# mym-br/gama_tts

Hardware: AMD Instinct MI355X
Metric: audio samples/sec (whole node), batched VTM @44.1kHz (higher is better)
Workload: dtype f32

## Files before the change

__graft_entry__.py:

```python
import os
import subprocess
import sys

ROOT = os.path.dirname(os.path.abspath(__file__))
for p in (ROOT, os.path.join(ROOT, "tests")):
    if p not in sys.path:
        sys.path.insert(0, p)


def build():
    env = dict(os.environ)
    subprocess.run(["make", "-C", os.path.join(ROOT, "gama_tts_amd", "csrc"), "ARCH=gfx950"], check=True, env=env)
    subprocess.run(["make", "-C", os.path.join(ROOT, "oracle"), "oracle"], check=True, env=env)
    subprocess.run(["make", "-C", os.path.join(ROOT, "oracle"), "ref"], check=True, env=env)
    import gama_tts_amd

    gama_tts_amd.load_library()


def smoke():
    import numpy as np

    import gama_tts_amd as g
    import oracle
    import tracks

    params = tracks.random_tracks(4, 25, seed0=42, consonant_heavy=True)
    cfgd = g.read_config_file(oracle.VOICE_MALE)
    plan = g.Plan(g.config_from_dict(cfgd, 44100.0, 1), 250.0, 0)
    audio, counts, maxabs = plan.synthesize_host(params)
    ref = oracle.synthesize_batch(oracle.male_config(44100.0, 1), params)
    assert audio.shape == ref.shape and (counts == ref.shape[1]).all(), (audio.shape, ref.shape, counts)
    err = float(np.abs(audio.astype(np.float64) - ref).max() / np.abs(ref).max())
    assert err < 2e-7, err
    assert np.allclose(maxabs, np.abs(audio).max(axis=1))
    from gama_tts_amd import capi
    plan32 = g.Plan(g.config_from_dict(cfgd, 44100.0, 1, capi.PRECISION_F32), 250.0, 0)
    audio32, _, _ = plan32.synthesize_host(params)
    ref32 = oracle.synthesize_batch(oracle.male_config(44100.0, 1, float_model=1), params)
    assert np.array_equal(audio32, ref32)
    plan5 = g.Plan(g.config5_from_dict(g.read_config_file(oracle.VOICE5_MALE)), 250.0, 0)
    audio5, counts5, _ = plan5.synthesize_host(params[:2])
    err5 = 0.0
    for b in range(2):
        ref5, _ = oracle.synthesize5(oracle.male5_config(48000.0), params[b])
        assert counts5[b] == ref5.size
        err5 = max(err5, float(np.abs(audio5[b, : ref5.size].astype(np.float64) - ref5).max() / np.abs(ref5).max()))
    assert err5 < 2e-6, err5
    plan5f = g.Plan(g.config5_from_dict(g.read_config_file(oracle.VOICE5_MALE), None, capi.PRECISION_F32), 250.0, 0, float_model5=True)
    audio5f, counts5f, _ = plan5f.synthesize_host(params[:2])
    for b in range(2):
        ref5f, _ = oracle.synthesize5(oracle.male5_config(48000.0, 1), params[b])
        assert counts5f[b] == ref5f.size and np.array_equal(audio5f[b, : ref5f.size], ref5f)
    print("smoke ok: batch=4 frames=25 samples=%d fp64 peak-relative error %.3g, float path bit-identical, model 5 error %.3g, "
          "float model 5 bit-identical" % (ref.shape[1], err, err5))


if __name__ == "__main__":
    build()
    if len(sys.argv) > 1 and sys.argv[1] == "smoke":
        smoke()
```

gama_tts_amd/capi.py:

```python
import ctypes
import os

import numpy as np

_HERE = os.path.dirname(os.path.abspath(__file__))
_LIB_NAME = "libgama_vtm.so"
N_PARAM = 16
DEVICE_NONE = -1
PRECISION_F64 = 0
PRECISION_MIXED = 1
PRECISION_F32 = 2
TUBE_10_6 = 0
TUBE_30_18 = 1
TABLE_FIR, TABLE_SRC_H, TABLE_SRC_DH, TABLE_WAVETABLE = 0, 1, 2, 3
_STATUS_UNSUPPORTED = 4


class GvtmError(RuntimeError):
    def __init__(self, status, message):
        super().__init__("gvtm status %d: %s" % (status, message))
        self.status = status


class Config(ctypes.Structure):
# ... 118 lines not shown
        "gvtm_plan_reserve": (i, [vp, sz]),
        "gvtm_host_alloc": (i, [sz, vp]),
        "gvtm_host_free": (None, [vp]),
        "gvtm_stream_create": (i, [vp, sz, vp]),
        "gvtm_stream_create_voices": (i, [vp, vp, sz, vp]),
        "gvtm_stream_destroy": (None, [vp]),
        "gvtm_stream_reset": (i, [vp]),
        "gvtm_stream_reset_voices": (i, [vp, vp]),
        "gvtm_stream_capacity": (sz, [vp, sz]),
        "gvtm_stream_push": (i, [vp, vp, vp, sz, vp, sz, vp]),
        "gvtm_stream_finish": (i, [vp, vp, sz, vp, vp]),
        "gvtm_normalize_batch_device": (i, [vp, vp, sz, sz, vp, vp, vp, vp, vp, vp]),
        "gvtm_plan_set_timing": (i, [vp, i]),
        "gvtm_plan_take_kernel_ms": (dbl, [vp, vp]),
        "gvtm_tracks_frame_count": (sz, [tracks, vp, sz]),
        "gvtm_generate_tracks_device": (i, [i, tracks, vp, vp, sz, sz, vp, vp, vp, vp]),
        "gvtm_synthesize_events_device": (i, [vp, tracks, vp, vp, sz, sz, vp, sz, vp, vp, vp, vp, vp]),
        "gvtm_plan_set_voice_tracks": (i, [vp, tracks, sz]),
        "gvtm_generate_tracks_voices_device": (i, [vp, vp, vp, vp, sz, sz, vp, vp, vp, vp]),
        "gvtm_synthesize_events_voices_device": (i, [vp, vp, vp, vp, sz, sz, vp, sz, vp, vp, vp, vp, vp]),
        "gvtm_tracks_chunks_frame_count": (sz, [tracks, vp, vp, sz]),
        "gvtm_generate_tracks_chunks_device": (i, [vp, vp, vp, vp, vp, sz, sz, vp, vp, vp, vp]),
        "gvtm_synthesize_events_chunks_device": (i, [vp, vp, vp, vp, vp, sz, sz, vp, sz, vp, vp, vp, vp, vp]),
        "gvtm_intonation_apply_host": (i64, [tracks, vp, sz, vp, sz, vp, sz, vp]),
        "gvtm_apply_intonation_device": (i, [vp, vp, vp, sz, vp, vp, vp, vp, sz, vp, sz, vp, vp, vp]),
        "gvtm_synthesize_intonation_device": (i, [vp, vp, vp, sz, vp, vp, vp, vp, sz, sz, sz, vp, sz, vp, vp, vp, vp, vp, vp]),
        "gvtm_modification_filter_length": (i64, [vp, i]),
        "gvtm_modification_apply_host": (i, [vp, i, vp, sz, vp, vp, sz, vp, vp, vp, vp]),
        "gvtm_apply_modifications_device": (i, [vp, vp, vp, sz, vp, vp, vp, vp, vp, vp, vp, sz, sz, vp, vp, vp, vp]),
        "gvtm_synthesize_modified_device": (i, [vp, vp, vp, sz, vp, vp, vp, vp, vp, vp, vp, sz, sz, vp, sz, vp, vp, vp, vp, vp]),
        "gvtm_targets_filter_length": (i64, [vp, i]),
        "gvtm_targets_output_count": (sz, [vp, sz]),
        "gvtm_targets_output_capacity": (sz, [vp, sz]),
        "gvtm_targets_apply_host": (i, [vp, i, vp, vp, vp, i64, vp, vp]),
        "gvtm_targets_apply_host_from": (i, [vp, i, vp, vp, vp, i64, i64, vp, vp, vp]),
        "gvtm_synthesize_targets_device": (i, [vp, vp, sz, vp, vp, vp, vp, sz, sz, vp, sz, vp, vp, vp, vp]),
        "gvtm_stream_push_targets": (i, [vp, vp, vp, vp, vp, sz, vp, sz, vp, vp]),
        "gvtm_stream_targets_capacity": (sz, [vp, sz]),
        "gvtm_stream_targets_points": (i, [vp, vp]),
        "gvtm_stream_push_events": (i, [vp, vp, vp, vp, vp, sz, vp, vp]),
        "gvtm_stream_get_drift": (i, [vp, vp]),
        "gvtm_stream_set_drift": (i, [vp, vp]),
        "gvtm_events_packed_layout": (sz, [vp, vp, vp, vp, vp, sz, vp, vp]),
        "gvtm_synthesize_events_packed_host": (i, [vp, vp, vp, vp, vp, sz, vp, sz, vp, vp, vp, sz, vp, vp, vp]),
        "gvtm_synthesize_events_packed_host_pcm16": (i, [vp, vp, vp, vp, vp, sz, vp, sz, vp, vp, vp, sz, vp, vp, vp, vp]),
        "gvtm_generate_tracks_host": (i, [i, tracks, vp, vp, sz, sz, vp, vp, vp]),
    }
    hooks = {
        "gvtm_debug_set_rows": (i, [vp, i]),
        "gvtm_debug_lds_bytes": (sz, [vp, i]),
        "gvtm_debug_launch_shape": (i, [vp, sz, i, vp]),
        "gvtm_debug_stream_launch_shape": (i, [vp, sz, vp]),
        "gvtm_debug_chunk_length": (i, [vp, sz]),
        "gvtm_debug_fir_literals": (i, [vp]),
        "gvtm_debug_plan_fir_literals": (i, [vp]),
        "gvtm_debug_force_generic_fir": (i, [vp]),
        "gvtm_debug_plan_src_phases": (i, [vp]),
        "gvtm_debug_plan_src_phase_table": (i, [vp, vp, sz]),
        "gvtm_debug_force_generic_src": (i, [vp]),
        "gvtm_debug_plan_static_wavetable": (i, [vp]),
        "gvtm_debug_force_dynamic_wavetable": (i, [vp]),
        "gvtm_debug_noise_table": (i, [sz, i, vp]),
        "gvtm_debug_set_taps": (i, [vp, vp]),
        "gvtm_debug_set_phase_cycles": (i, [vp, vp]),
        "gvtm_debug_dpp_selftest": (i, [vp, vp]),
        "gvtm_debug_short_math": (i, [i, vp, sz, vp]),
        "gvtm_debug_device_float_math": (i, [vp, i, vp, sz, vp]),
        "gvtm_debug_group_voices": (i, [vp, vp, sz, i, vp, vp, vp, vp]),
        "gvtm_debug_tracks_append": (i, [vp, vp, vp, vp, vp, vp, sz, sz, vp, vp, vp]),
        "gvtm_debug_tracks_slice": (i, [vp, vp, i64, vp, vp, vp, vp, sz, sz, vp, vp, vp, vp]),
        "gvtm_debug_carry_rows": (i, [vp, vp, vp, vp, sz, sz]),
    }
    return product, hooks


PROTOTYPES, HOOK_PROTOTYPES = _prototypes()
_REQUIRED = (
    "gvtm_status_string", "gvtm_last_error", "gvtm_device_count", "gvtm_plan_create", "gvtm_plan_create_model5", "gvtm_plan_destroy",
    "gvtm_plan_info", "gvtm_plan_table", "gvtm_output_count", "gvtm_output_capacity", "gvtm_synthesize_batch_device",
    "gvtm_synthesize_batch_host", "gvtm_synthesize_batch_host_pcm16", "gvtm_host_alloc", "gvtm_host_free", "gvtm_normalize_batch_device",
    "gvtm_tracks_frame_count", "gvtm_generate_tracks_device", "gvtm_synthesize_events_device", "gvtm_generate_tracks_host",
    "gvtm_stream_create", "gvtm_stream_destroy", "gvtm_stream_reset", "gvtm_stream_capacity", "gvtm_stream_push", "gvtm_stream_finish",
    "gvtm_plan_set_timing", "gvtm_plan_take_kernel_ms")


def library_path(diagnostics=False):
    return os.path.join(_HERE, "lib", "libgama_vtm_diag.so" if diagnostics else _LIB_NAME)


_libs = {}


def load_library(diagnostics=False):
    if diagnostics in _libs:
        return _libs[diagnostics]
    path = (os.environ.get("GVTM_DIAG_LIBRARY") or library_path(True)) if diagnostics else (os.environ.get("GVTM_LIBRARY") or library_path())
    try:
        import torch
    except ImportError:
        pass
    if not os.path.exists(path):
        raise ImportError("%s is missing: run `python -c 'import __graft_entry__ as g; g.build()'` "
                          "(make -C gama_tts_amd/csrc). There is no fallback path." % path)
    lib = ctypes.CDLL(path)
    table = {**PROTOTYPES, **HOOK_PROTOTYPES} if diagnostics else PROTOTYPES
    for name, (restype, argtypes) in table.items():
# ... 286 lines not shown
            _check(self._lib, rc)

    def close(self):
        if self._h:
            self._lib.gvtm_plan_destroy(self._h)
            self._h = ctypes.c_void_p()

    def __del__(self):
        try:
            self.close()
        except Exception:
            pass

    def table(self, which):
        buf = np.empty(4096, dtype=np.float64)
        n = self._lib.gvtm_plan_table(self._h, which, buf.ctypes.data, buf.size)
        if n < 0:
            self._check(-n)
        return buf[:n].copy()

    def uses_fir_literals(self):
        rc = self._lib.gvtm_debug_plan_fir_literals(self._h)
        if rc < 0:
            self._check(-rc)
        return bool(rc)

    def force_generic_fir(self):
        self._check(self._lib.gvtm_debug_force_generic_fir(self._h))

    def _hook_count(self, rc):
        if rc < 0:
            self._check(-rc)
        return int(rc)

    def src_phases(self):
        return self._hook_count(self._lib.gvtm_debug_plan_src_phases(self._h))

    def src_phase_table(self):
        phases = self.src_phases()
        if not phases:
            return None
        out = np.empty((phases, 28), dtype=np.float32)
        assert self._hook_count(self._lib.gvtm_debug_plan_src_phase_table(self._h, out.ctypes.data, out.size)) == phases
        return out

    def force_generic_src(self):
        self._check(self._lib.gvtm_debug_force_generic_src(self._h))

    def says_static_wavetable(self):
        return bool(self._hook_count(self._lib.gvtm_debug_plan_static_wavetable(self._h)))

    def force_dynamic_wavetable(self):
        self._check(self._lib.gvtm_debug_force_dynamic_wavetable(self._h))

    def output_count(self, frames):
        return int(self._lib.gvtm_output_count(self._h, int(frames)))

    def output_capacity(self, max_frames):
        return int(self._lib.gvtm_output_capacity(self._h, int(max_frames)))

    def set_timing(self, enabled):
        self._check(self._lib.gvtm_plan_set_timing(self._h, int(bool(enabled))))

    def take_kernel_ms(self):
        n = ctypes.c_int(0)
        ms = self._lib.gvtm_plan_take_kernel_ms(self._h, ctypes.byref(n))
        return float(ms), int(n.value)

    def synthesize_device(self, d_params, batch, max_frames, d_audio, audio_stride, d_frame_counts=None,
                          d_out_counts=None, d_maxabs=None, stream=None):
        self._check(self._lib.gvtm_synthesize_batch_device(
            self._h, _ptr(d_params), _ptr(d_frame_counts), int(batch), int(max_frames), _ptr(d_audio),
            int(audio_stride), _ptr(d_out_counts), _ptr(d_maxabs), _ptr(stream)))

    @staticmethod
    def _host_outputs(batch, shape, dtype):
        return (np.zeros(shape, dtype=dtype), np.zeros(batch, dtype=np.int64), np.zeros(batch, dtype=np.float32),
                np.zeros(batch, dtype=np.float32) if dtype == np.int16 else None)

    def _host(self, params, frame_counts, dtype):
        params = np.ascontiguousarray(params, dtype=np.float32)
        assert params.ndim == 3 and params.shape[2] == N_PARAM
        batch, frames = params.shape[:2]
        assert frame_counts is None or np.shape(frame_counts) == (batch,)
        stride = self.output_count(frames) if frame_counts is None else self.output_capacity(frames)
        out, counts, maxabs, scales = self._host_outputs(batch, (batch, stride), dtype)
        self.synthesize_host_into(params, out, frame_counts, counts, maxabs, scales)
        return out, counts, maxabs, scales

    def synthesize_host(self, params, frame_counts=None):
        return self._host(params, frame_counts, np.float32)[:3]

    def synthesize_host_pcm16(self, params, frame_counts=None):
        return self._host(params, frame_counts, np.int16)

    def synthesize_host_into(self, params, out, frame_counts=None, counts=None, maxabs=None, scales=None):
        assert params.dtype == np.float32 and params.flags.c_contiguous and params.ndim == 3 and params.shape[2] == N_PARAM
        assert out.flags.c_contiguous and out.ndim == 2 and out.shape[0] == params.shape[0]
        batch, frames = params.shape[:2]
        fc = None
        if frame_counts is not None:
            fc = np.ascontiguousarray(frame_counts, dtype=np.int32)
        if out.dtype == np.int16:
            self._check(self._lib.gvtm_synthesize_batch_host_pcm16(
                self._h, _ptr(params), _ptr(fc), batch, frames, _ptr(out), out.shape[1], _ptr(counts), _ptr(maxabs), _ptr(scales)))
        else:
# ... 384 lines not shown
```

gama_tts_amd/csrc/vtm_capi_hooks.cpp:

```cpp
#include <cstring>

#include "vtm_host.hpp"
#include "vtm_math.hpp"

using namespace gvtm::host;

static int finish_kernel(hipError_t launched, const char* what)
{
	const hipError_t e = launched == hipSuccess ? hipDeviceSynchronize() : launched;
	return e == hipSuccess ? GVTM_OK : fail_hip(e, what);
}

extern "C" {

#pragma GCC visibility push(default)

int gvtm_debug_set_rows(gvtm_plan* plan, int rows)
{
	if (!plan) return fail(GVTM_ERR_INVALID_ARGUMENT, "null plan");
	plan->rows = rows;
	return GVTM_OK;
}

size_t gvtm_debug_lds_bytes(const gvtm_plan* plan, int rows)
{
	if (!plan) return 0;
	return gvtm::synth_launch_shape(plan->designs.data(), 1, plan->precision, 0, rows, false, 0, false).lds;
}

int gvtm_debug_launch_shape(const gvtm_plan* plan, size_t batch, int voices, size_t out[3])
{
	if (!plan || !out) return fail(GVTM_ERR_INVALID_ARGUMENT, "null plan or buffer");
	const gvtm::LaunchShape shape = plan->launch_shape(batch, 0, voices != 0);
	if (!shape.rows) return fail(GVTM_ERR_UNSUPPORTED, "LDS budget exceeded");
	out[0] = static_cast<size_t>(shape.rows), out[1] = static_cast<size_t>(shape.ring), out[2] = shape.lds;
	return GVTM_OK;
}

int gvtm_debug_stream_launch_shape(const gvtm_plan* plan, size_t batch, size_t out[3])
{
	if (!plan || !out) return fail(GVTM_ERR_INVALID_ARGUMENT, "null plan or buffer");
	if (plan->designs[0].model5) return fail(GVTM_ERR_UNSUPPORTED, "a plan of the models 0 to 4");
	const gvtm::LaunchShape shape = plan->stream_launch_shape(batch, 0, plan->longest_stream_ring());
	if (!shape.rows) return fail(GVTM_ERR_UNSUPPORTED, "LDS budget exceeded");
	out[0] = static_cast<size_t>(shape.rows), out[1] = static_cast<size_t>(shape.ring), out[2] = shape.lds;
	return GVTM_OK;
}

int gvtm_debug_chunk_length(const gvtm_plan* plan, size_t batch)
{
	if (!plan) return -fail(GVTM_ERR_INVALID_ARGUMENT, "null plan");
	if (plan->designs[0].model5) return 0;
	const gvtm::LaunchShape shape = plan->launch_shape(batch, 0, false);
	if (!shape.rows) return 0;
	return gvtm::synth_chunk_length(plan->designs[0].k, plan->precision, shape.rows);
}

int gvtm_debug_fir_literals(float* out)
{
	if (!out) return fail(GVTM_ERR_INVALID_ARGUMENT, "null buffer");
	std::memcpy(out, gvtm::kGlottalFirF32, sizeof(gvtm::kGlottalFirF32));
	return gvtm::kGlottalFirTapsF32;
}

int gvtm_debug_plan_fir_literals(const gvtm_plan* plan)
{
	if (!plan) return -fail(GVTM_ERR_INVALID_ARGUMENT, "null plan");
	return plan->fir_literals ? 1 : 0;
}

int gvtm_debug_force_generic_fir(gvtm_plan* plan)
{
	if (!plan) return fail(GVTM_ERR_INVALID_ARGUMENT, "null plan");
	plan->fir_literals = false;
	return GVTM_OK;
}

int gvtm_debug_plan_src_phases(const gvtm_plan* plan)
{
	if (!plan) return -fail(GVTM_ERR_INVALID_ARGUMENT, "null plan");
	return static_cast<int>(plan->src_phases);
}

int gvtm_debug_plan_src_phase_table(const gvtm_plan* plan, float* out, size_t capacity)
{
	if (!plan || !out) return -fail(GVTM_ERR_INVALID_ARGUMENT, "null plan or buffer");
	if (!plan->src_phases) return 0;
	const std::vector<float> table = gvtm::design_src_phase_table(plan->designs[0]);
	if (capacity < table.size()) return -fail(GVTM_ERR_INVALID_ARGUMENT, "table buffer too small");
	std::memcpy(out, table.data(), sizeof(float) * table.size());
	return static_cast<int>(plan->src_phases);
}

int gvtm_debug_force_generic_src(gvtm_plan* plan)
{
	if (!plan) return fail(GVTM_ERR_INVALID_ARGUMENT, "null plan");
	plan->src_phases = 0;
	return GVTM_OK;
}

int gvtm_debug_plan_static_wavetable(const gvtm_plan* plan)
{
	if (!plan) return -fail(GVTM_ERR_INVALID_ARGUMENT, "null plan");
	return plan->static_wavetable ? 1 : 0;
}

int gvtm_debug_force_dynamic_wavetable(gvtm_plan* plan)
{
// ... 139 lines not shown
```

gama_tts_amd/csrc/vtm_kernel_v2.inc:

```

namespace v2 {

namespace {

constexpr int kPrm = 17;
constexpr int kF1Planes = 6;
constexpr int kF1U = 0, kF1Sig = 1, kF1Thr = 2, kF1B0 = 3, kF1A1 = 4, kF1A2 = 5;
constexpr int kKl = 11;
constexpr int kKlK8 = 7, kKlNk1 = 8, kKlAlr = 9, kKlAu = 10;
constexpr int kInj = 9;
template <typename CT, int LAYOUT>
constexpr bool lane_rec()
{
	return sizeof(CT) == 4 && LAYOUT == 0;
}
constexpr int kLrZero = 16, kLrAlr = 17, kLrAu = 18, kLrK8 = 19, kLrKn = 20, kLrInj = 21, kLrLen = 31;
constexpr int kl_len(bool lr)
{
	return lr ? kLrLen : kKl;
}
template <typename CT>
constexpr bool fr_compact()
{
	return sizeof(CT) == 8;
}
template <typename CT>
constexpr int fr_len()
{
	return fr_compact<CT>() ? 5 : 9;
}
constexpr int kFrTapA = 0, kFrTapB = 1, kFrZero = 2, kFrFirst = 3;
template <int C>
constexpr int rec_pad(int rec)
{
	return ((16 - (C * rec) % 32) + 32) % 32;
}
template <int C, int U>
constexpr int rec_slot(int rec)
{
	return U * C * rec + rec_pad<C>(rec) * ((U + 1) / 2);
}
template <int C, int U>
__host__ __device__ constexpr size_t rec_at(int rec, int slot, int u)
{
	return static_cast<size_t>(slot) * rec_slot<C, U>(rec) + static_cast<size_t>(u) * (C * rec) + static_cast<size_t>(rec_pad<C>(rec)) * ((u + 1) / 2);
}
constexpr int kDump = 64 * 4;
constexpr int kXMirror = 32;
constexpr int kWPre = 48;
static_assert(kWPre == kStreamPreRoll, "a stream state carries one pre-roll");

struct Extent {
	int frames;
	int nchunks;
	uint32_t steps;
	int last_frame;
	unsigned long long step_base;
	unsigned long long k_first;
};

#ifndef GVTM_KERNEL_TAPS
#define GVTM_KERNEL_TAPS 0
#endif
#ifndef GVTM_TUNE_SKIP
#define GVTM_TUNE_SKIP 0
#endif
#ifndef GVTM_TUNE_TRACE
#define GVTM_TUNE_TRACE 0
#endif
#ifndef GVTM_TUNE_PLAN_TABLES
#define GVTM_TUNE_PLAN_TABLES (-1)
#endif
constexpr unsigned kSerialHelpMask = 0x1a;
template <typename CT, typename ST, int U>
constexpr bool kSrcHOnly = sizeof(ST) == 8 && U > 1;
template <typename CT, typename ST, int U, int C>
struct Smem {
	DeviceConstants* kc;
	Extent* ext;
	CT* wavetable;
	CT* fir;
	SrcTap<ST>* src;
	float* prm;
	CT* inc;
	CT* amp;
	CT* pos;
	CT* noise;
	CT* w;
	CT* usg;
	CT* fr;
	CT* kl;
	CT* inj;
	CT* lanec;
	CT* thy;
	CT* ox;
	CT* opk;
	ST* x;
	unsigned* peak;
	unsigned long long* kb;
	unsigned* ticket;
	unsigned long long* diag;
	CT* dump;
};

template <typename CT, typename ST, int U, int C, bool LR>
struct SmemOffsets {
	size_t kc, ext, wavetable, fir, src, prm, inc, amp, pos, noise, w, usg, fr, kl, inj, lanec, thy, ox, opk, peak, kb, ticket, diag, dump, x, fixed;
	__host__ __device__ constexpr SmemOffsets()
		: kc(0), ext(0), wavetable(0), fir(0), src(0), prm(0), inc(0), amp(0), pos(0), noise(0), w(0), usg(0), fr(0), kl(0),
		  inj(0), lanec(0), thy(0), ox(0), opk(0), peak(0), kb(0), ticket(0), diag(0), dump(0), x(0), fixed(0)
	{
		size_t off = 0;
		auto take = [&](size_t bytes) {
			const size_t at = off;
			off += (bytes + 15) & ~size_t(15);
			return at;
		};
		kc = take(sizeof(DeviceConstants));
		ext = take(sizeof(Extent) * U);
		wavetable = take(sizeof(CT) * kWavetableLength);
		fir = take(sizeof(CT) * kMaxFirTaps);
		src = take(kSrcHOnly<CT, ST, U> ? sizeof(ST) * (kSrcFilterLength + 1) : sizeof(SrcTap<ST>) * kSrcFilterLength);
		prm = take(sizeof(float) * 2 * rec_slot<C, U>(kPrm));
		inc = take(sizeof(CT) * 2 * U * C);
// ... 115 lines not shown
			{kJunction, -1, 0, 0, -1},
			{kCopy, kKlNk1, 0, 1, -1},
			c,
			{kJunction, -1, 0, 0, -1},
			{kCopy, -1, 2, 1, -1},
			c,
			{kJunction, -1, 0, 0, -1},
			{kCopy, -1, 3, 1, -1},
			c,
			{kJunction, -1, 0, 0, -1},
			{kCopy, -1, 4, 1, -1},
			c,
			{kJunction, -1, 0, 0, -1},
			{kCopy, -1, 5, 1, -1},
			c,
			{kEnd, -1, 0, 0, -1},
		};
		return t[L < 48 ? L : 47];
	}
};

}

template <int U, int LAYOUT>
constexpr int serial_waves()
{
	return TubeLayout<LAYOUT>::kWaveWide ? U + 4 : 5 * ((U + 3) / 4);
}

constexpr int kVoicesFlag = 2;
constexpr int kTargetsFlag = 4;

__device__ __forceinline__ size_t voice_row(const SynthArgs& a, size_t slot)
{
	const int r = a.row_map[slot];
	return r < 0 ? a.batch : static_cast<size_t>(r);
}

template <int D, int U> constexpr bool far_calls_inline() { return D == 1 && U == 4; }
template <int D, int U> constexpr bool fir_literal_taps() { return !((D == 1 && U == 1) || (D == 2 && U == 2)); }
template <typename CT, int D, int U, int LAYOUT> constexpr bool bounds_by_recurrence() { return sizeof(CT) == 4 && U == 4 && LAYOUT == 0 && (D == 2 || D == 3); }
template <typename CT, int D, int U, int LAYOUT, bool VOICES> constexpr bool src_phase_table()
{
	constexpr bool can = sizeof(CT) == 4 && !VOICES;
	if (GVTM_TUNE_PLAN_TABLES >= 0) return can && (GVTM_TUNE_PLAN_TABLES & 1) != 0;
	return can && LAYOUT == 0 && ((U == 4 && D == 1) || (U == 2 && D == 2));
}
template <typename CT, int D, int U, int LAYOUT, bool VOICES> constexpr bool static_wavetable_pass()
{
	constexpr bool can = sizeof(CT) == 4 && !VOICES;
	if (GVTM_TUNE_PLAN_TABLES >= 0) return can && (GVTM_TUNE_PLAN_TABLES & 2) != 0;
	return can && LAYOUT == 0 && ((U == 4 && (D == 1 || D == 2)) || (U == 2 && D == 2));
}
template <typename CT, int D, int U, bool VOICES> constexpr bool float_arg_consts() { return sizeof(CT) == 4 && !VOICES && !far_calls_inline<D, U>(); }

template <typename CT, typename ST, int D, int U, int C, int NH, int LAYOUT_FLAGS>
__global__ __launch_bounds__((serial_waves<U, LAYOUT_FLAGS & 1>() + NH) * 64) void vtm_synth_kernel(const SynthArgs a)
{
	constexpr int LAYOUT = LAYOUT_FLAGS & 1;
	constexpr bool VOICES = (LAYOUT_FLAGS & kVoicesFlag) != 0;
	constexpr bool TARGETS = (LAYOUT_FLAGS & kTargetsFlag) != 0;
	static_assert(!(TARGETS && VOICES), "targets: one voice");
	int voice = 0;
	if constexpr (VOICES) {
		voice = a.group_voice[blockIdx.x];
		if (voice < 0) return;
	}
	using TL = TubeLayout<LAYOUT>;
	static_assert(!TL::kWaveWide || U <= 4, "wave-wide tubes: one tube wavefront per utterance, at most four");
	constexpr int kSerial = serial_waves<U, LAYOUT>();
	static_assert(C % D == 0, "chunk must be a multiple of the section delay");
	static_assert(U == 1 || U == 2 || U == 4 || U == 8, "utterances per workgroup = DPP rows used");
	constexpr int G = (U + 3) / 4;
	static_assert(2 * C >= kWPre, "FIR pre-roll copy needs 2C >= kWPre");
	const int XR = VOICES ? synth_ring_for(a.kconst[voice].upsampling, a.kconst[voice].pad, a.stream ? a.stream_chunk : C) : a.xr;
	const int XRS = XR + kXMirror;
	static_assert(NH >= 1, "at least one helper wavefront");
	constexpr int kThreads = (kSerial + NH) * 64;

	extern __shared__ __attribute__((aligned(16))) unsigned char smem_raw[];
	constexpr bool kLaneRec = lane_rec<CT, LAYOUT>();
	constexpr SmemOffsets<CT, ST, U, C, kLaneRec> so;
	Smem<CT, ST, U, C> sm;
	sm.kc = reinterpret_cast<DeviceConstants*>(smem_raw + so.kc);
	sm.ext = reinterpret_cast<Extent*>(smem_raw + so.ext);
	sm.wavetable = reinterpret_cast<CT*>(smem_raw + so.wavetable);
	sm.fir = reinterpret_cast<CT*>(smem_raw + so.fir);
	sm.src = reinterpret_cast<SrcTap<ST>*>(smem_raw + so.src);
	sm.prm = reinterpret_cast<float*>(smem_raw + so.prm);
	sm.inc = reinterpret_cast<CT*>(smem_raw + so.inc);
	sm.amp = reinterpret_cast<CT*>(smem_raw + so.amp);
	sm.pos = reinterpret_cast<CT*>(smem_raw + so.pos);
	sm.noise = reinterpret_cast<CT*>(smem_raw + so.noise);
	sm.w = reinterpret_cast<CT*>(smem_raw + so.w);
	sm.usg = reinterpret_cast<CT*>(smem_raw + so.usg);
	sm.fr = reinterpret_cast<CT*>(smem_raw + so.fr);
	sm.kl = reinterpret_cast<CT*>(smem_raw + so.kl);
	sm.inj = reinterpret_cast<CT*>(smem_raw + so.inj);
	sm.lanec = reinterpret_cast<CT*>(smem_raw + so.lanec);
	sm.thy = reinterpret_cast<CT*>(smem_raw + so.thy);
	sm.ox = reinterpret_cast<CT*>(smem_raw + so.ox);
	sm.opk = reinterpret_cast<CT*>(smem_raw + so.opk);
	sm.x = reinterpret_cast<ST*>(smem_raw + so.x);
	sm.peak = reinterpret_cast<unsigned*>(smem_raw + so.peak);
	sm.dump = reinterpret_cast<CT*>(smem_raw + so.dump);
	sm.diag = reinterpret_cast<unsigned long long*>(smem_raw + so.diag);
	sm.ticket = reinterpret_cast<unsigned*>(smem_raw + so.ticket);
	sm.kb = reinterpret_cast<unsigned long long*>(smem_raw + so.kb);

	const int tid = threadIdx.x;
	const int lane = tid & 63;
	const int wave = tid >> 6;
	const int hl = lane;
	const size_t group = blockIdx.x;
#define GVTM_ROW_UTT(u, ...) (VOICES ? voice_row(a, group * U + (u)) : __VA_ARGS__)
	constexpr bool kArgConsts = float_arg_consts<CT, D, U, VOICES>();
	constexpr bool kFarInline = far_calls_inline<D, U>();
#define GVTM_KF(idx, field) (kArgConsts ? static_cast<CT>(a.fir_k.f[kFirKConsts + (idx)]) : CT(k.field))
	constexpr int kFr = fr_len<CT>();
	constexpr bool kFrCompact = fr_compact<CT>();
	auto at_prm = [](int slot, int u) { return rec_at<C, U>(kPrm, slot, u); };
	auto at_usg = [](int slot, int u) { return rec_at<C, U>(kF1Planes, slot, u); };
	auto at_fr = [](int slot, int u) { return rec_at<C, U>(fr_len<CT>(), slot, u); };
	constexpr bool kMaskedSerial = sizeof(ST) == 4;
	constexpr int kStaticRounds = (U == 4 && LAYOUT == 0 && (sizeof(CT) == 4 || (sizeof(ST) == 8 ? D <= 2 : D == 1))) ? 1 : 0;
	constexpr bool kHelperByRole = sizeof(CT) == 4 || D >= 3 || (sizeof(ST) == 8 && D == 2);
	constexpr bool kNoiseTable = sizeof(CT) == 4;
	constexpr bool kBoundsRecurrence = bounds_by_recurrence<CT, D, U, LAYOUT>();
	constexpr bool kSrcPhaseTable = src_phase_table<CT, D, U, LAYOUT, VOICES>();
	constexpr bool kStaticWavetablePass = static_wavetable_pass<CT, D, U, LAYOUT, VOICES>();
	constexpr int kKlLen = kl_len(kLaneRec);
	constexpr int kInjLen = kLaneRec ? kKlLen : kInj;
	auto at_kl = [](int slot, int u) { return rec_at<C, U>(kKlLen, slot, u); };
	constexpr bool kBlockRec = kLaneRec && D != 3;
	auto kl_index = [](int s, int e) -> int {
		if constexpr (kBlockRec) return (s >> 2) * (kKlLen * 4) + e * 4 + (s & 3);
		else return s * kKlLen + e;
	};
	auto at_inj = [](int slot, int u) { return kLaneRec ? rec_at<C, U>(kKlLen, slot, u) + kLrInj : rec_at<C, U>(kInj, slot, u); };
	auto amp_at = [](int slot, int u, int which, int s) -> size_t {
		return ((static_cast<size_t>(slot) * U + u) * 2 + which) * C + s;
	};
	const bool kPush = a.stream_mode == kStreamPush;
	const bool kFinal = !kPush;
	using SL = StreamLayout<CT, ST>;
	constexpr int kTubeLanes = TubeLayout<LAYOUT>::kLanes;
	constexpr int kTubeWords = 2 * D + 1;

	{
		const int* src = reinterpret_cast<const int*>(VOICES ? a.kconst + voice : a.kconst);
		int* dst = reinterpret_cast<int*>(sm.kc);
		for (int i = tid; i < static_cast<int>(sizeof(DeviceConstants) / sizeof(int)); i += kThreads) dst[i] = src[i];
	}
	for (int i = tid; i < kWavetableLength; i += kThreads) sm.wavetable[i] = VOICES ? static_cast<const CT*>(a.wavetable)[static_cast<size_t>(voice) * kWavetableLength + i] : static_cast<const CT*>(a.wavetable)[i];
	for (int i = tid; i < kSrcFilterLength; i += kThreads) {
		if constexpr (kSrcHOnly<CT, ST, U>) {
			reinterpret_cast<ST*>(sm.src)[i] = static_cast<ST>(static_cast<const CT*>(a.src_h)[i]);
			if (i == 0) reinterpret_cast<ST*>(sm.src)[kSrcFilterLength] = ST(0);
		} else {
			sm.src[i].h = static_cast<ST>(static_cast<const CT*>(a.src_h)[i]);
			sm.src[i].dh = static_cast<ST>(static_cast<const CT*>(a.src_dh)[i]);
		}
	}
	for (int i = tid; i < 3 * U * (kWPre + 2 * C); i += kThreads) sm.w[i] = CT(0.0);
	for (int i = tid; i < U * XRS; i += kThreads) sm.x[i] = ST(0);
	__syncthreads();
	if (tid < U) {
		Extent e{0, 0, 0, 0, 0ull, 0ull};
		const size_t ug = GVTM_ROW_UTT(tid, group * U + tid);
		unsigned peak0 = 0u;
		if (ug < a.batch) {
			const size_t rows_avail = a.max_frames - (kPush && !TARGETS ? 1 : 0);
			const int f = a.frame_counts ? a.frame_counts[ug] : static_cast<int>(rows_avail);
			e.frames = f > 0 ? (static_cast<size_t>(f) < rows_avail ? f : static_cast<int>(rows_avail)) : 0;
			e.steps = TARGETS ? static_cast<uint32_t>(e.frames) : static_cast<uint32_t>(e.frames) * sm.kc->control_steps;
			e.nchunks = e.steps == 0 ? 1 : static_cast<int>((e.steps + C - 1) / C);
			e.last_frame = e.frames - 1 + (kPush ? 1 : 0);
			if (a.stream) {
				const StreamHeader* h = reinterpret_cast<const StreamHeader*>(a.stream + ug * a.stream_stride);
				e.step_base = h->step_base;
				e.k_first = ((e.step_base << 16) + sm.kc->time_inc - 1) / sm.kc->time_inc;
				peak0 = h->peak_bits;
			}
// ... 824 lines not shown
			}
			return r;
		};
		CT injv[kB];
		auto step = [&](const Blk& r, int q, CT& x1, CT& x2, CT& y1, CT& y2, int s, CT& thy_out) {
			const CT fric = rmul(r.b0[q], r.sig[q] - x2) - rmul(r.a1[q], y1) - rmul(r.a2[q], y2);
			x2 = r.sig[q]; y2 = fric;
			const CT ty = rmul(tb0, r.thr[q]) - rmul(ta1, thr_y1);
			thr_y1 = ty;
			if constexpr (kBlockRec) injv[q] = (Lf == 0) ? r.u[q] : r.tap[q] * fric;
			else inj_w[inj_stride * s] = (Lf == 0) ? r.u[q] : r.tap[q] * fric;
			thy_out = ty * tgain;
		};
		if (valid > 0) {
			auto process = [&](const Blk& cb, int s0) {
				CT ty[kB];
#pragma unroll
				for (int q = 0; q < kB; q += 2) {
					step(cb, q, bp_x1, bp_x2, bp_y1, bp_y2, s0 + q, ty[q]);
					step(cb, q + 1, bp_x2, bp_x1, bp_y2, bp_y1, s0 + q + 1, ty[q + 1]);
				}
				if constexpr (kBlockRec) {
					using F4 = float __attribute__((ext_vector_type(4)));
					static_assert(!kBlockRec || (kB == 4 && kMaskedSerial), "block layout: float, blocks of four steps, owning lanes only");
					*reinterpret_cast<F4*>(sm.kl + at_kl(c & 1, u) + kl_index(s0, kLrInj + Lf)) = F4{injv[0], injv[1], injv[2], injv[3]};
				}
				CT* tw = thy_w + thy_stride * s0;
				if (!kMaskedSerial || Lf == 0) {
#pragma unroll
					for (int q = 0; q < kB; ++q) tw[thy_stride ? q : 0] = ty[q];
				}
			};
			if constexpr (kBlockRec) {
				Blk ba = fetch(0);
				int s0 = 0;
				for (; s0 + kB < valid; s0 += 2 * kB) {
					const Blk bb = fetch(s0 + kB);
					process(ba, s0);
					ba = fetch(s0 + 2 * kB);
					process(bb, s0 + kB);
				}
				if (s0 < valid) process(ba, s0);
			} else {
				Blk nb = fetch(0);
				for (int s0 = 0; s0 < valid; s0 += kB) {
					const Blk cb = nb;
					nb = fetch(s0 + kB);
					process(cb, s0);
				}
			}
		}
	};

	auto stage_f2 = [&](int c) {
		const int u = urow;
		const int valid = valid_in(u, c);
		if (valid < 0) return;
		const Extent e = sm.ext[u];
		const bool active = U >= 4 || row < U;
		const uint32_t n0 = static_cast<uint32_t>(e.step_base) + static_cast<uint32_t>(c) * C;
		const CT* ox = sm.ox + (static_cast<size_t>(c & 1) * U + u) * C * 2;
		const CT* thy = sm.thy + (static_cast<size_t>(c % 3) * U + u) * C;
		ST* xr = sm.x + u * XRS;
		const int which = L == 0 ? 0 : 1;
		const CT ra = L == 0 ? GVTM_KF(kKfMouthARad, mouth_a_rad) : GVTM_KF(kKfNoseARad, nose_a_rad);
		const bool x_owner = active && L == 0;
		ST* const x_dump = reinterpret_cast<ST*>(sm.dump + 128 + lane);
		const bool dbg = GVTM_KERNEL_TAPS && a.debug_taps != nullptr && active && L == 0;
		if (kMaskedSerial && !(active && L < 2)) {
		} else {
		const CT* po = ox + which * C;
		const CT* pt = thy;
		const CT* pq = kLaneRec ? sm.opk + (static_cast<size_t>(c % 3) * U + u) * C : thy;
		const CT opk_nose = CT(1.0) + GVTM_KF(kKfNasalK5, nasal_k[5]);
		static_assert(C % 4 == 0, "post-tube filters work in blocks of four steps");
		struct Blk2 { CT x[4], t[4], q[4]; };
		auto fetch2 = [&]() {
			Blk2 r;
#pragma unroll
			for (int q = 0; q < 4; ++q) { r.x[q] = po[q]; r.t[q] = pt[q]; if constexpr (kLaneRec) r.q[q] = pq[q]; }
			po += 4; pt += 4; pq += 4;
			return r;
		};
		auto process2 = [&](const Blk2& cb, int s0) {
			ST out[4];
#pragma unroll
			for (int q = 0; q < 4; ++q) {
				CT xin = cb.x[q];
				if constexpr (kLaneRec) xin = rmul(L == 0 ? cb.q[q] : opk_nose, xin);
				const CT oy = (rmul(ra, xin) - rmul(ra, rad_x1)) + rmul(ra, rad_y1);
				rad_x1 = xin; rad_y1 = oy;
				CT sample = oy + from_right(oy);
				sample += cb.t[q];
				out[q] = static_cast<ST>(sample);
				if (dbg) a.debug_taps[(GVTM_ROW_UTT(u, (group * U + u)) * a.max_frames * k.control_steps + static_cast<uint32_t>(c) * C + s0 + q) * 8 + 7] = sample;
			}
			const unsigned slot = (n0 + s0) & (XR - 1);
			ST* xw = x_owner ? xr + slot : x_dump;
#pragma unroll
			for (int q = 0; q < 4; ++q) xw[q] = out[q];
			ST* xm = (x_owner && slot < static_cast<unsigned>(kXMirror)) ? xr + XR + slot : x_dump + 4;
#pragma unroll
			for (int q = 0; q < 4; ++q) xm[q] = out[q];
		};
		if constexpr (kBlockRec) {
			Blk2 ba = fetch2();
			int s0 = 0;
			for (; s0 + 4 < valid; s0 += 8) {
				const Blk2 bb = fetch2();
				process2(ba, s0);
				ba = fetch2();
				process2(bb, s0 + 4);
			}
			if (s0 < valid) process2(ba, s0);
		} else {
			Blk2 nb = fetch2();
			for (int s0 = 0; s0 < valid; s0 += 4) {
				const Blk2 cb = nb;
				nb = fetch2();
				process2(cb, s0);
			}
		}
// ... 513 lines not shown
```

gama_tts_amd/csrc/vtm_kernels.hip:

```cpp
#include <hip/hip_runtime.h>

#include <algorithm>
#include <cstdint>
#include <type_traits>

#include "vtm_design.hpp"
#include "vtm_kernels.hpp"
#include "vtm_math.hpp"

namespace gvtm {

namespace {
#include "vtm_device_common.inc"
}

#include "vtm_kernel_v2.inc"
#include "vtm_kernel_m5.inc"

__global__ __launch_bounds__(256) void vtm_normalize_kernel(const NormalizeArgs a)
{
	const size_t utt = blockIdx.y;
	const int64_t n = a.counts ? a.counts[utt] : static_cast<int64_t>(a.audio_stride);
	const float peak = a.maxabs[utt];
	const float scale = (peak < 1.0e-30f) ? 0.0f : 0.95f / peak;
	if (a.scales && blockIdx.x == 0 && threadIdx.x == 0) a.scales[utt] = scale;
	const float* __restrict__ in = a.audio + utt * a.audio_stride;
	const int64_t limit = n < static_cast<int64_t>(a.audio_stride) ? n : static_cast<int64_t>(a.audio_stride);
	for (int64_t i = static_cast<int64_t>(blockIdx.x) * blockDim.x + threadIdx.x; i < limit;
			i += static_cast<int64_t>(gridDim.x) * blockDim.x) {
		const float v = in[i] * scale;
		if (a.out_f32) a.out_f32[utt * a.audio_stride + i] = v;
		if (a.out_i16) a.out_i16[utt * a.audio_stride + i] = static_cast<int16_t>(static_cast<int>(roundf(v * 32767.0f)));
	}
}

#include "vtm_kernel_shapes.hpp"

template <typename S, bool VOICES>
static hipError_t launch_v2(const SynthArgs& args, size_t batch, hipStream_t stream)
{
	if constexpr (VOICES && S::U == 8) {
		return hipErrorInvalidValue;
	} else {
		auto fn = v2::vtm_synth_kernel<typename S::CT, typename S::ST, S::D, S::U, S::C, S::NH, S::LAYOUT | (VOICES ? v2::kVoicesFlag : 0)>;
		if (args.xr < ring_length(args.k, S::C) || (args.xr & (args.xr - 1)) != 0 || 2 * S::C + 4 * args.k.pad + 64 > args.xr) return hipErrorInvalidValue;
		if (!args.k.upsampling && args.xr != kSrcRing) return hipErrorInvalidValue;
		if constexpr (v2::float_arg_consts<typename S::CT, S::D, S::U, VOICES>()) {
			if (args.fir_k.f[kFirKConsts + kKfBasicIncrement] != static_cast<float>(args.k.basic_increment)) return hipErrorInvalidValue;
		}
		const size_t lds = S::lds_bytes(args.xr);
		hipError_t e = hipFuncSetAttribute(reinterpret_cast<const void*>(fn), hipFuncAttributeMaxDynamicSharedMemorySize,
				static_cast<int>(lds));
		if (e != hipSuccess) return e;
		const unsigned groups = static_cast<unsigned>(VOICES ? batch : (batch + S::U - 1) / S::U);
		hipLaunchKernelGGL(fn, dim3(groups), dim3(S::kWaves * 64), lds, stream, args);
		return hipGetLastError();
	}
}

hipError_t launch_synth(const SynthArgs& args, size_t batch, int precision, int rows, hipStream_t stream)
{
	const auto launch = [&](auto voices) {
		return with_shape(precision, rows, args.k.section_delay, args.k.layout, hipErrorInvalidValue,
				[&](auto s) { return launch_v2<decltype(s), decltype(voices)::value>(args, batch, stream); });
	};
	if (args.tg_offsets) return args.row_map ? hipErrorInvalidValue : launch_synth_targets(args, batch, precision, rows, stream);
	if (!args.row_map) return launch(std::false_type{});
	if (!args.group_voice) return hipErrorInvalidValue;
	return launch(std::true_type{});
}

int synth_chunk_length(const DeviceConstants& k, int precision, int rows)
{
	return with_shape(precision, rows, k.section_delay, k.layout, 0, [](auto s) { return decltype(s)::C; });
}

size_t stream_state_bytes(const DeviceConstants& k, int precision, int xr)
{
	const int lanes = k.layout == 1 ? 48 : 16, words = 2 * k.section_delay + 1;
	return with_shape(precision, 1, k.section_delay, k.layout, size_t(0), [&](auto s) {
		return StreamLayout<typename decltype(s)::CT, typename decltype(s)::ST>::bytes(lanes, words, xr);
	});
}

static LaunchShape shape_of_rows(const DeviceConstants& k, int precision, int rows, int xr)
{
	return with_shape(precision, rows, k.section_delay, k.layout, LaunchShape{}, [&](auto s) {
		using S = decltype(s);
		const int ring = xr > 0 ? xr : ring_length(k, S::C);
		return LaunchShape{S::U, ring, S::lds_bytes(ring), S::U, S::U};
	});
}

LaunchShape synth_launch_shape(const Design* voices, int n_voices, int precision, size_t batch, int forced_rows, bool several_voices,
		int stream_ring, bool fit)
{
	const auto fits = [&](const LaunchShape& s) { return !fit || s.lds <= kLdsPerWorkgroup; };
	if (voices[0].model5) {
		const bool float_class = precision == GVTM_PRECISION_F32;
		const int index = float_class ? (forced_rows == 1 ? 0 : (forced_rows == 2 || batch > 256 ? 1 : 0)) : (forced_rows == 2 && !several_voices ? 1 : 0);
		const M5Shape m = m5_shape(float_class, index);
		const size_t lds = float_class ? synth5_float_lds_bytes(index) : (index == 1 ? m5_lds_bytes<false, 1>() : m5_lds_bytes<false, 0>());
		const LaunchShape s{m.rows, 0, lds, index + 1, m.rows * m.groups_per_cu};
		return fits(s) ? s : LaunchShape{};
	}
	int rows = forced_rows;
	if (rows != 1 && rows != 2 && rows != 4 && rows != 8) {
		rows = batch > 512 ? 4 : (batch > 256 ? 2 : 1);
		if (precision != GVTM_PRECISION_F32 && voices[0].k.section_delay >= 3 && rows > 2) rows = 2;
	}
	if (rows > 4 && (precision != GVTM_PRECISION_F32 || several_voices)) rows = 4;
	for (;; rows /= 2) {
		int ring = stream_ring;
		for (int v = 0; !stream_ring && v < n_voices; ++v) ring = std::max(ring, shape_of_rows(voices[v].k, precision, rows, 0).ring);
		const LaunchShape s = shape_of_rows(voices[0].k, precision, rows, ring);
		if (s.rows == 0 || fits(s)) return s;
		if (s.rows == 1) return LaunchShape{};
		rows = s.rows;
	}
}

constexpr int kGroupThreads = kGroupVoicesThreads;
__global__ __launch_bounds__(kGroupThreads) void vtm_group_voices_kernel(const GroupVoicesArgs a)
{
	constexpr int T = kGroupThreads;
	__shared__ int scan[T];
	const int t = threadIdx.x;
// ... 72 lines not shown
```

gama_tts_amd/csrc/vtm_kernels.hpp:

```cpp
#pragma once

#include <hip/hip_runtime.h>

#include <cstddef>
#include <cstdint>

#include "vtm_design.hpp"
#include "vtm_targets.hpp"

namespace gvtm {

struct StreamHeader {
	unsigned long long step_base;
	double seed;
	unsigned peak_bits;
	unsigned reserved_;
	unsigned long long pad_;
};
static_assert(sizeof(StreamHeader) == 32, "stream header layout");
constexpr int kStreamScalars = 12;
constexpr int kSsPos = 0, kSsPrev = 1;
constexpr int kSsBp = 2, kSsThr = 6;
constexpr int kSsRadMouth = 7, kSsRadNose = 9;
constexpr int kStreamPreRoll = 48;
// ... 58 lines not shown
	double* debug_taps;
	unsigned long long* phase_cycles;
	const Model5Constants* k5const = nullptr;
	const int32_t* row_map = nullptr;
	const int32_t* group_voice = nullptr;
	int stream_chunk = 0;
	int fir_literals = 0;
	const float* src_phase = nullptr;
	unsigned src_phase_mask = 0;
	int static_wavetable = 0;
	const int64_t* tg_offsets = nullptr;
	const int32_t* tg_ids = nullptr;
	const int32_t* tg_steps = nullptr;
	const float* tg_values = nullptr;
	int64_t tg_N = 0;
	double tg_invN = 0.0;
};

struct GroupVoicesArgs {
	const int32_t* voice_ids;
	size_t batch;
	int n_voices;
	int rows;
	size_t groups;
	int32_t* row_map;
	int32_t* group_voice;
	int32_t* counts;
	int64_t* out_counts;
	float* maxabs;
};
constexpr int kGroupVoicesThreads = 256;

struct NormalizeArgs {
	const float* audio;
	const int64_t* counts;
	const float* maxabs;
	float* out_f32;
	int16_t* out_i16;
	float* scales;
	size_t audio_stride;
};

struct LaunchShape {
	int rows = 0;
	int ring = 0;
	size_t lds = 0;
	int forced = 0;
	int per_cu = 0;
};
constexpr size_t kLdsPerWorkgroup = 160 * 1024;
LaunchShape synth_launch_shape(const Design* voices, int n_voices, int precision, size_t batch, int forced_rows, bool several_voices,
		int stream_ring = 0, bool fit = true);
int synth_chunk_length(const DeviceConstants& k, int precision, int rows);
hipError_t launch_synth(const SynthArgs& args, size_t batch, int precision, int rows, hipStream_t stream);
hipError_t launch_synth_targets(const SynthArgs& args, size_t batch, int precision, int rows, hipStream_t stream);
size_t stream_state_bytes(const DeviceConstants& k, int precision, int xr);
hipError_t launch_group_voices(const GroupVoicesArgs& args, hipStream_t stream);
hipError_t launch_synth5(const SynthArgs& args, size_t batch, int precision, int index, hipStream_t stream);
hipError_t launch_synth5_float(const SynthArgs& args, size_t batch, int index, hipStream_t stream);
size_t synth5_float_lds_bytes(int index);
hipError_t launch_synth5_voices(const SynthArgs& args, size_t groups, hipStream_t stream);
hipError_t launch_synth5_float_voices(const SynthArgs& args, size_t groups, int index, hipStream_t stream);
constexpr int kDppSelftestInts = 640;
hipError_t launch_dpp_selftest(int* d_out , hipStream_t stream);
hipError_t launch_float_math_probe(int kind, const float* d_x, size_t n, float* d_out, hipStream_t stream);
hipError_t launch_normalize(const NormalizeArgs& args, size_t batch, hipStream_t stream);

}
```

Baseline: 17.29 billion.

## Split post-tube radiation filters into parallel FIR part and short serial recurrence

```diff
diff --git a/__graft_entry__.py b/__graft_entry__.py
--- a/__graft_entry__.py
+++ b/__graft_entry__.py
@@ -10,7 +10,7 @@
 
 def build():
     env = dict(os.environ)
-    subprocess.run(["make", "-C", os.path.join(ROOT, "gama_tts_amd", "csrc"), "ARCH=gfx950"], check=True, env=env)
+    subprocess.run(["make", "-j4", "-C", os.path.join(ROOT, "gama_tts_amd", "csrc"), "ARCH=gfx950"], check=True, env=env)
     subprocess.run(["make", "-C", os.path.join(ROOT, "oracle"), "oracle"], check=True, env=env)
     subprocess.run(["make", "-C", os.path.join(ROOT, "oracle"), "ref"], check=True, env=env)
     import gama_tts_amd
diff --git a/gama_tts_amd/capi.py b/gama_tts_amd/capi.py
--- a/gama_tts_amd/capi.py
+++ b/gama_tts_amd/capi.py
@@ -194,6 +194,7 @@
         "gvtm_debug_launch_shape": (i, [vp, sz, i, vp]),
         "gvtm_debug_stream_launch_shape": (i, [vp, sz, vp]),
         "gvtm_debug_chunk_length": (i, [vp, sz]),
+        "gvtm_debug_plan_filter_split": (i, [vp, i]),
         "gvtm_debug_fir_literals": (i, [vp]),
         "gvtm_debug_plan_fir_literals": (i, [vp]),
         "gvtm_debug_force_generic_fir": (i, [vp]),
@@ -586,6 +587,9 @@
 
     def force_dynamic_wavetable(self):
         self._check(self._lib.gvtm_debug_force_dynamic_wavetable(self._h))
+
+    def filter_split(self, rows):
+        return self._hook_count(self._lib.gvtm_debug_plan_filter_split(self._h, int(rows)))
 
     def output_count(self, frames):
         return int(self._lib.gvtm_output_count(self._h, int(frames)))
diff --git a/gama_tts_amd/csrc/vtm_capi_hooks.cpp b/gama_tts_amd/csrc/vtm_capi_hooks.cpp
--- a/gama_tts_amd/csrc/vtm_capi_hooks.cpp
+++ b/gama_tts_amd/csrc/vtm_capi_hooks.cpp
@@ -54,6 +54,13 @@
 	const gvtm::LaunchShape shape = plan->launch_shape(batch, 0, false);
 	if (!shape.rows) return 0;
 	return gvtm::synth_chunk_length(plan->designs[0].k, plan->precision, shape.rows);
+}
+
+int gvtm_debug_plan_filter_split(const gvtm_plan* plan, int rows)
+{
+	if (!plan) return -fail(GVTM_ERR_INVALID_ARGUMENT, "null plan");
+	if (plan->designs[0].model5) return 0;
+	return gvtm::synth_filter_split(plan->designs[0].k, plan->precision, rows);
 }
 
 int gvtm_debug_fir_literals(float* out)
diff --git a/gama_tts_amd/csrc/vtm_kernel_v2.inc b/gama_tts_amd/csrc/vtm_kernel_v2.inc
--- a/gama_tts_amd/csrc/vtm_kernel_v2.inc
+++ b/gama_tts_amd/csrc/vtm_kernel_v2.inc
@@ -70,6 +70,9 @@
 #endif
 #ifndef GVTM_TUNE_PLAN_TABLES
 #define GVTM_TUNE_PLAN_TABLES (-1)
+#endif
+#ifndef GVTM_TUNE_FILTER_SPLIT
+#define GVTM_TUNE_FILTER_SPLIT (-1)
 #endif
 constexpr unsigned kSerialHelpMask = 0x1a;
 template <typename CT, typename ST, int U>
@@ -291,6 +294,12 @@
 	if (GVTM_TUNE_PLAN_TABLES >= 0) return can && (GVTM_TUNE_PLAN_TABLES & 2) != 0;
 	return can && LAYOUT == 0 && ((U == 4 && (D == 1 || D == 2)) || (U == 2 && D == 2));
 }
+template <typename CT, typename ST, int D, int U, int LAYOUT, bool VOICES> constexpr bool filter_split_f2()
+{
+	constexpr bool can = sizeof(CT) == 4 && sizeof(ST) == 4 && LAYOUT == 0 && D != 3 && !VOICES;
+	if (GVTM_TUNE_FILTER_SPLIT >= 0) return can && (GVTM_TUNE_FILTER_SPLIT & 1) != 0;
+	return can && U == 4 && D == 2;
+}
 template <typename CT, int D, int U, bool VOICES> constexpr bool float_arg_consts() { return sizeof(CT) == 4 && !VOICES && !far_calls_inline<D, U>(); }
 
 template <typename CT, typename ST, int D, int U, int C, int NH, int LAYOUT_FLAGS>
@@ -368,6 +377,7 @@
 	constexpr bool kBoundsRecurrence = bounds_by_recurrence<CT, D, U, LAYOUT>();
 	constexpr bool kSrcPhaseTable = src_phase_table<CT, D, U, LAYOUT, VOICES>();
 	constexpr bool kStaticWavetablePass = static_wavetable_pass<CT, D, U, LAYOUT, VOICES>();
+	constexpr bool kSplitF2 = filter_split_f2<CT, ST, D, U, LAYOUT, VOICES>();
 	constexpr int kKlLen = kl_len(kLaneRec);
 	constexpr int kInjLen = kLaneRec ? kKlLen : kInj;
 	auto at_kl = [](int slot, int u) { return rec_at<C, U>(kKlLen, slot, u); };
@@ -1298,9 +1308,112 @@
 		}
 	};
 
+	auto stage_f2_split = [&]([[maybe_unused]] int c, [[maybe_unused]] int valid) {
+		if constexpr (kSplitF2) {
+#pragma clang fp contract(off)
+		using F4 = float __attribute__((ext_vector_type(4)));
+		static_assert(!kSplitF2 || (kBlockRec && kMaskedSerial && kRowView && C % 4 == 0), "split post-tube filters: float, block record, row view");
+		constexpr int kRows = U < 4 ? U : 4;
+		const int ub = U >= 4 ? sub * 4 : 0;
+		CT* const oxs = sm.ox + (static_cast<size_t>(c & 1) * U + ub) * C * 2;
+		const CT* const opks = sm.opk + (static_cast<size_t>(c % 3) * U + ub) * C;
+		const CT* const thys = sm.thy + (static_cast<size_t>(c % 3) * U + ub) * C;
+		const CT ra_m = GVTM_KF(kKfMouthARad, mouth_a_rad), ra_n = GVTM_KF(kKfNoseARad, nose_a_rad);
+		const CT opk_nose = CT(1.0) + GVTM_KF(kKfNasalK5, nasal_k[5]);
+		int ln = lane;
+		asm volatile("" : "+v"(ln));
+		const int L = ln & 15, row = ln >> 4;
+		const bool owner = (U >= 4 || row < U) && L < 2 && valid > 0;
+		CT x_last = CT(0.0);
+		if (owner) x_last = rmul(L == 0 ? opks[row * C + valid - 1] : opk_nose, oxs[(row * 2 + L) * C + valid - 1]);
+		CT* const lds0 = reinterpret_cast<CT*>(smem_raw);
+		unsigned ix = static_cast<unsigned>(oxs - lds0) + ln, iq = static_cast<unsigned>(opks - lds0) + ln, it = static_cast<unsigned>(thys - lds0) + ln;
+		const int back = ln > 0 ? 1 : 0;
+		unsigned ixb = ix - back, iqb = iq - back;
+		asm volatile("" : "+v"(ix), "+v"(iq), "+v"(it), "+v"(ixb), "+v"(iqb));
+		CT* const px = lds0 + ix;
+		const CT* const pq = lds0 + iq;
+		const CT* const pt = lds0 + it;
+		const CT* const pxb = lds0 + ixb;
+		const CT* const pqb = lds0 + iqb;
+#pragma unroll
+		for (int sb = ((C - 1) / 64) * 64; sb >= 0; sb -= 64) {
+			if (C - sb < 64 && ln >= C - sb) continue;
+			const CT* const pxl = sb > 0 ? px - 1 : pxb;
+			const CT* const pql = sb > 0 ? pq - 1 : pqb;
+			const bool left = sb > 0 || ln > 0;
+#pragma unroll
+			for (int r = 0; r < 2 * kRows; ++r) {
+				const int o = r * C + sb;
+				const CT x = px[o], xp = pxl[o];
+				CT p, pp;
+				if (r & 1) {
+					p = rmul(ra_n, rmul(opk_nose, x)); pp = rmul(ra_n, rmul(opk_nose, xp));
+				} else {
+					const int oq = (r >> 1) * C + sb;
+					p = rmul(ra_m, rmul(pq[oq], x)); pp = rmul(ra_m, rmul(pql[oq], xp));
+				}
+				px[o] = left ? p - pp : p;
+			}
+		}
+		__builtin_amdgcn_fence(__ATOMIC_ACQ_REL, "wavefront");
+		if (owner) {
+			const CT ra = L == 0 ? ra_m : ra_n;
+			unsigned id = static_cast<unsigned>(oxs + (row * 2 + L) * C - lds0);
+			asm volatile("" : "+v"(id));
+			F4* pd = reinterpret_cast<F4*>(lds0 + id);
+			CT y1 = rad_y1;
+			auto run = [&](const F4& d) {
+				F4 y;
+				y.x = d.x + rmul(ra, y1);
+				y.y = d.y + rmul(ra, y.x);
+				y.z = d.z + rmul(ra, y.y);
+				y.w = d.w + rmul(ra, y.z);
+				y1 = y.w;
+				return y;
+			};
+			F4 da = pd[0];
+			da.x = da.x - rmul(ra, rad_x1);
+			int s0 = 0;
+			for (; s0 + 4 < valid; s0 += 8) {
+				const F4 db = pd[1];
+				pd[0] = run(da);
+				da = pd[2];
+				pd[1] = run(db);
+				pd += 2;
+			}
+			if (s0 < valid) pd[0] = run(da);
+			rad_x1 = x_last;
+			rad_y1 = y1;
+		}
+		__builtin_amdgcn_fence(__ATOMIC_ACQ_REL, "wavefront");
+		const bool dbg = GVTM_KERNEL_TAPS && a.debug_taps != nullptr;
+#pragma unroll
+		for (int sb = 0; sb < C; sb += 64) {
+			if (C - sb < 64 && ln >= C - sb) continue;
+			const int s = sb + ln;
+#pragma unroll
+			for (int r = 0; r < kRows; ++r) {
+				const int uu = ub + r;
+				const CT sample = (px[2 * r * C + sb] + px[(2 * r + 1) * C + sb]) + pt[r * C + sb];
+				if (s < valid_in(uu, c)) {
+					const unsigned slot = (static_cast<uint32_t>(sm.ext[uu].step_base) + static_cast<uint32_t>(c) * C + s) & (XR - 1);
+					ST* xr = sm.x + uu * XRS;
+					xr[slot] = static_cast<ST>(sample);
+					if (slot < static_cast<unsigned>(kXMirror)) xr[XR + slot] = static_cast<ST>(sample);
+					if (dbg) a.debug_taps[(GVTM_ROW_UTT(uu, (group * U + uu)) * a.max_frames * k.control_steps + static_cast<uint32_t>(c) * C + s) * 8 + 7] = sample;
+				}
+			}
+		}
+		}
+	};
+
 	auto stage_f2 = [&](int c) {
 		const int u = urow;
 		const int valid = valid_in(u, c);
+		if constexpr (kSplitF2) {
+			if (c >= 0 && c < max_chunks) stage_f2_split(c, valid);
+		}
 		if (valid < 0) return;
 		const Extent e = sm.ext[u];
 		const bool active = U >= 4 || row < U;
@@ -1313,7 +1426,7 @@
 		const bool x_owner = active && L == 0;
 		ST* const x_dump = reinterpret_cast<ST*>(sm.dump + 128 + lane);
 		const bool dbg = GVTM_KERNEL_TAPS && a.debug_taps != nullptr && active && L == 0;
-		if (kMaskedSerial && !(active && L < 2)) {
+		if (kSplitF2 || (kMaskedSerial && !(active && L < 2))) {
 		} else {
 		const CT* po = ox + which * C;
 		const CT* pt = thy;
diff --git a/gama_tts_amd/csrc/vtm_kernels.hip b/gama_tts_amd/csrc/vtm_kernels.hip
--- a/gama_tts_amd/csrc/vtm_kernels.hip
+++ b/gama_tts_amd/csrc/vtm_kernels.hip
@@ -73,6 +73,14 @@
 int synth_chunk_length(const DeviceConstants& k, int precision, int rows)
 {
 	return with_shape(precision, rows, k.section_delay, k.layout, 0, [](auto s) { return decltype(s)::C; });
+}
+
+int synth_filter_split(const DeviceConstants& k, int precision, int rows)
+{
+	return with_shape(precision, rows, k.section_delay, k.layout, 0, [](auto s) {
+		using S = decltype(s);
+		return v2::filter_split_f2<typename S::CT, typename S::ST, S::D, S::U, S::LAYOUT, false>() ? 1 : 0;
+	});
 }
 
 size_t stream_state_bytes(const DeviceConstants& k, int precision, int xr)
diff --git a/gama_tts_amd/csrc/vtm_kernels.hpp b/gama_tts_amd/csrc/vtm_kernels.hpp
--- a/gama_tts_amd/csrc/vtm_kernels.hpp
+++ b/gama_tts_amd/csrc/vtm_kernels.hpp
@@ -134,6 +134,7 @@
 LaunchShape synth_launch_shape(const Design* voices, int n_voices, int precision, size_t batch, int forced_rows, bool several_voices,
 		int stream_ring = 0, bool fit = true);
 int synth_chunk_length(const DeviceConstants& k, int precision, int rows);
+int synth_filter_split(const DeviceConstants& k, int precision, int rows);
 hipError_t launch_synth(const SynthArgs& args, size_t batch, int precision, int rows, hipStream_t stream);
 hipError_t launch_synth_targets(const SynthArgs& args, size_t batch, int precision, int rows, hipStream_t stream);
 size_t stream_state_bytes(const DeviceConstants& k, int precision, int xr);
```

Measured after the change: 17.53 billion, median of 6. 1.01x the previous value.
